# kkoutini/PaSST

Measured on AMD Instinct MI355X. Metric: clips/s (10s@32k) fwd+bwd passt_s, higher is better.
Workload: dtype bf16; 1 GPU; passt_s_swa_p16_128_ap476 train step (mel front end + mixup + fwd + BCE + bwd + adamw), 768/12/12, 474 tokens (s_patchout_t=40,f=4), random-init weights; global_batch=64, per_gpu_batch=64, parallelism=dp1, gemm_launch=persistent, 256 workgroups, input=waveform (B,1,320000) f32 resident in HBM

## Files before the change

### passt_amd/csrc/layernorm.hip

```cpp
#include <algorithm>
#include <cstdlib>

#include "pa_common.h"

namespace pa {

static constexpr int LN_MAXV = 8;
static constexpr int LN_BWD_BLOCKS = 1024;

__device__ __forceinline__ float4 ldrow4(const float* p) {
    return *(const float4*)p;
}
template <typename T> __device__ __forceinline__ void store4(T* p, const float4& v);
template <> __device__ __forceinline__ void store4<float>(float* p, const float4& v) {
    *(float4*)p = v;
}
template <> __device__ __forceinline__ void store4<bf16>(bf16* p, const float4& v) {
    bf16x4 o; o[0] = (bf16)v.x; o[1] = (bf16)v.y; o[2] = (bf16)v.z; o[3] = (bf16)v.w;
    *(bf16x4*)p = o;
}
template <typename T> __device__ __forceinline__ float4 load4(const T* p);
template <> __device__ __forceinline__ float4 load4<float>(const float* p) { return ldrow4(p); }
template <> __device__ __forceinline__ float4 load4<bf16>(const bf16* p) {
    const bf16x4 v = *(const bf16x4*)p;
    return make_float4((float)v[0], (float)v[1], (float)v[2], (float)v[3]);
}

template <typename T, int MAXV>
__global__ __launch_bounds__(256) void ln_fwd_kernel(const float* __restrict__ x, const float* __restrict__ gamma,
                                                     const float* __restrict__ beta, T* __restrict__ y,
                                                     float* __restrict__ mean, float* __restrict__ rstd,
                                                     int M, int D, float eps) {
    const int lane = threadIdx.x & 63;
    const int row = blockIdx.x * 4 + (threadIdx.x >> 6);
    if (row >= M) return;
    const int nv = D >> 2;
    const float* xr = x + (int64_t)row * D;
    float4 v[MAXV];
    float s = 0.f;
#pragma unroll
    for (int i = 0; i < MAXV; ++i) {
        const int c = lane + 64 * i;
        if (c < nv) { v[i] = ldrow4(xr + 4 * c); s += (v[i].x + v[i].y) + (v[i].z + v[i].w); }
    }
    const float mu = wave_sum(s) / (float)D;
    float s2 = 0.f;
#pragma unroll
    for (int i = 0; i < MAXV; ++i) {
        const int c = lane + 64 * i;
        if (c < nv) {
            const float a = v[i].x - mu, b = v[i].y - mu, cc = v[i].z - mu, d = v[i].w - mu;
            s2 += (a * a + b * b) + (cc * cc + d * d);
        }
    }
    const float r = rsqrtf(wave_sum(s2) / (float)D + eps);
    if (lane == 0) {
        if (mean) mean[row] = mu;
        if (rstd) rstd[row] = r;
    }
    T* yr = y + (int64_t)row * D;
#pragma unroll
    for (int i = 0; i < MAXV; ++i) {
        const int c = lane + 64 * i;
        if (c < nv) {
            const float4 g = *(const float4*)(gamma + 4 * c), b = *(const float4*)(beta + 4 * c);
            float4 o;
            o.x = (v[i].x - mu) * r * g.x + b.x; o.y = (v[i].y - mu) * r * g.y + b.y;
            o.z = (v[i].z - mu) * r * g.z + b.z; o.w = (v[i].w - mu) * r * g.w + b.w;
            store4<T>(yr + 4 * c, o);
        }
    }
}

template <typename T, int MAXV, bool ADD2>
__device__ __forceinline__ void ln_bwd_body(const T* __restrict__ dy, const float* __restrict__ x,
                                                     const float* __restrict__ gamma, const float* __restrict__ mean,
                                                     const float* __restrict__ rstd, const float* __restrict__ dres,
                                                     const float* __restrict__ dres2,
                                                     float* __restrict__ dx, T* __restrict__ dx_lp,
                                                     float* __restrict__ ws, int M, int D, float* red) {
    const int lane = threadIdx.x & 63, wave = threadIdx.x >> 6;
    const int nv = D >> 2;
    float4 g[MAXV], ag[MAXV], ab[MAXV], ac[MAXV];
#pragma unroll
    for (int i = 0; i < MAXV; ++i) {
        const int c = lane + 64 * i;
        g[i] = c < nv ? *(const float4*)(gamma + 4 * c) : make_float4(0, 0, 0, 0);
        ag[i] = make_float4(0, 0, 0, 0);
        ab[i] = make_float4(0, 0, 0, 0);
        ac[i] = make_float4(0, 0, 0, 0);
    }
    for (int row = blockIdx.x * 4 + wave; row < M; row += gridDim.x * 4) {
        const float mu = mean[row], r = rstd[row];
        const int64_t base = (int64_t)row * D;
        float4 xh[MAXV], gy[MAXV];
        float s1 = 0.f, s2 = 0.f;
#pragma unroll
        for (int i = 0; i < MAXV; ++i) {
            const int c = lane + 64 * i;
            if (c < nv) {
                const float4 xv = ldrow4(x + base + 4 * c);
                const float4 d = load4<T>(dy + base + 4 * c);
                xh[i] = make_float4((xv.x - mu) * r, (xv.y - mu) * r, (xv.z - mu) * r, (xv.w - mu) * r);
                gy[i] = make_float4(d.x * g[i].x, d.y * g[i].y, d.z * g[i].z, d.w * g[i].w);
                s1 += (gy[i].x + gy[i].y) + (gy[i].z + gy[i].w);
                s2 += (gy[i].x * xh[i].x + gy[i].y * xh[i].y) + (gy[i].z * xh[i].z + gy[i].w * xh[i].w);
                ag[i].x += d.x * xh[i].x; ag[i].y += d.y * xh[i].y; ag[i].z += d.z * xh[i].z; ag[i].w += d.w * xh[i].w;
                ab[i].x += d.x; ab[i].y += d.y; ab[i].z += d.z; ab[i].w += d.w;
            }
        }
        const float c1 = wave_sum(s1) / (float)D, c2 = wave_sum(s2) / (float)D;
#pragma unroll
        for (int i = 0; i < MAXV; ++i) {
            const int c = lane + 64 * i;
            if (c < nv) {
                float4 o;
                o.x = r * (gy[i].x - c1 - xh[i].x * c2); o.y = r * (gy[i].y - c1 - xh[i].y * c2);
                o.z = r * (gy[i].z - c1 - xh[i].z * c2); o.w = r * (gy[i].w - c1 - xh[i].w * c2);
                if (dres) {
                    const float4 dr = ldrow4(dres + base + 4 * c);
                    o.x += dr.x; o.y += dr.y; o.z += dr.z; o.w += dr.w;
                }
                if (ADD2) {
                    const float4 dr = ldrow4(dres2 + base + 4 * c);
                    o.x += dr.x; o.y += dr.y; o.z += dr.z; o.w += dr.w;
                }
                {
                    *(float4*)(dx + base + 4 * c) = o;
                }
                if (dx_lp) store4<T>(dx_lp + base + 4 * c, o);
                ac[i].x += o.x; ac[i].y += o.y; ac[i].z += o.z; ac[i].w += o.w;
            }
        }
    }
#pragma unroll
    for (int i = 0; i < MAXV; ++i) {
        const int c = lane + 64 * i;
        if (c < nv) {
            *(float4*)(red + (wave * 3 + 0) * D + 4 * c) = ag[i];
            *(float4*)(red + (wave * 3 + 1) * D + 4 * c) = ab[i];
            *(float4*)(red + (wave * 3 + 2) * D + 4 * c) = ac[i];
        }
    }
    __syncthreads();
    for (int k = threadIdx.x; k < 3 * D; k += 256) {
        const int which = k / D, c = k - which * D;
        float s = 0.f;
#pragma unroll
        for (int w = 0; w < 4; ++w) s += red[(w * 3 + which) * D + c];
        ws[(int64_t)blockIdx.x * 3 * D + k] = s;
    }
}

template <typename T, int MAXV>
__global__ __launch_bounds__(256) void ln_bwd_kernel(const T* __restrict__ dy, const float* __restrict__ x,
                                                     const float* __restrict__ gamma, const float* __restrict__ mean,
                                                     const float* __restrict__ rstd, const float* __restrict__ dres,
                                                     float* __restrict__ dx, T* __restrict__ dx_lp,
                                                     float* __restrict__ ws, int M, int D) {
    extern __shared__ __attribute__((aligned(16))) float red[];
    ln_bwd_body<T, MAXV, false>(dy, x, gamma, mean, rstd, dres, nullptr, dx, dx_lp, ws, M, D, red);
}

template <typename T, int MAXV>
__global__ __launch_bounds__(256) void ln_bwd2_kernel(const T* __restrict__ dy, const float* __restrict__ x,
                                                      const float* __restrict__ gamma, const float* __restrict__ mean,
                                                      const float* __restrict__ rstd, const float* __restrict__ dres,
                                                      const float* __restrict__ dres2,
                                                      float* __restrict__ dx, T* __restrict__ dx_lp,
                                                      float* __restrict__ ws, int M, int D) {
    extern __shared__ __attribute__((aligned(16))) float red[];
    ln_bwd_body<T, MAXV, true>(dy, x, gamma, mean, rstd, dres, dres2, dx, dx_lp, ws, M, D, red);
}

__global__ __launch_bounds__(256) void ln_bwd_reduce_kernel(const float* __restrict__ ws, int nblk, int D,
                                                            float* __restrict__ dgamma, float* __restrict__ dbeta,
                                                            float* __restrict__ dcol, int accumulate) {
    __shared__ float red[16][17];
    const int cx = threadIdx.x & 15, ry = threadIdx.x >> 4;
    const int k = blockIdx.x * 16 + cx;
    const int nk = dcol ? 3 * D : 2 * D;
    float s = 0.f, s1 = 0.f, s2 = 0.f, s3 = 0.f;
    if (k < nk) {
        int b = ry;
        for (; b + 48 < nblk; b += 64) {
            s += ws[(int64_t)b * 3 * D + k];
            s1 += ws[(int64_t)(b + 16) * 3 * D + k];
            s2 += ws[(int64_t)(b + 32) * 3 * D + k];
            s3 += ws[(int64_t)(b + 48) * 3 * D + k];
        }
        for (; b < nblk; b += 16) s += ws[(int64_t)b * 3 * D + k];
    }
    s = (s + s1) + (s2 + s3);
    red[ry][cx] = s;
    __syncthreads();
    if (ry == 0 && k < nk) {
        s = 0.f;
#pragma unroll
        for (int y = 0; y < 16; ++y) s += red[y][cx];
        float* out = k < D ? dgamma + k : (k < 2 * D ? dbeta + (k - D) : dcol + (k - 2 * D));
        *out = (accumulate ? *out : 0.f) + s;
    }
}

}

using namespace pa;

extern "C" int pa_layernorm_fwd(const float* x, const float* gamma, const float* beta, void* y, int dtype,
                                float* mean, float* rstd, int M, int D, float eps, void* stream) {
    if (!x || !gamma || !beta || !y || M <= 0 || D <= 0) return PA_EINVAL;
    if (D % 4 || D > LN_MAXV * 256) return PA_EUNSUPPORTED;
    dim3 grid((unsigned)cdiv(M, 4));
    if (dtype != PA_BF16 && dtype != PA_F32) return PA_EINVAL;
    const int nvl = (int)cdiv(D, 256);
#define PA_LN_FWD(V)                                                                                              \
    do {                                                                                                          \
        if (dtype == PA_BF16) hipLaunchKernelGGL((ln_fwd_kernel<bf16, V>), grid, dim3(256), 0, (hipStream_t)stream, x, gamma, beta, (bf16*)y, mean, rstd, M, D, eps); \
        else hipLaunchKernelGGL((ln_fwd_kernel<float, V>), grid, dim3(256), 0, (hipStream_t)stream, x, gamma, beta, (float*)y, mean, rstd, M, D, eps); \
    } while (0)
    if (nvl <= 1) PA_LN_FWD(1); else if (nvl == 2) PA_LN_FWD(2); else if (nvl == 3) PA_LN_FWD(3);
    else if (nvl == 4) PA_LN_FWD(4); else PA_LN_FWD(8);
#undef PA_LN_FWD
    return check_launch();
}

static int ln_bwd_blocks(int M) {
    static const int cap = [] { const char* e = getenv("PA_LN_BWD_BLOCKS"); return e && atoi(e) > 0 ? atoi(e) : LN_BWD_BLOCKS; }();
    static const int rpw = [] { const char* e = getenv("PA_LN_BWD_ROWS_PER_WAVE"); return e && atoi(e) > 0 ? atoi(e) : 2; }();
    return (int)std::max<int64_t>(1, std::min<int64_t>(cap, cdiv(M, 4 * rpw)));
}

extern "C" int64_t pa_layernorm_bwd_ws_floats(int M, int D) { return (int64_t)ln_bwd_blocks(M) * 3 * D; }

extern "C" int pa_layernorm_bwd_rows(int M) { return M > 0 ? ln_bwd_blocks(M) : 0; }

static int ln_bwd_launch(const void* dy, int dtype, const float* x, const float* gamma, const float* mean, const float* rstd,
                         const float* dres, const float* dres2, float* dx, void* dx_lp, float* ws, int M, int D, hipStream_t st);

extern "C" int pa_layernorm_bwd_partial(const void* dy, int dtype, const float* x, const float* gamma,
                                        const float* mean, const float* rstd, const float* dres, float* dx,
                                        void* dx_lp, float* ws, int M, int D, void* stream) {
    if (!dy || !x || !gamma || !mean || !rstd || !dx || !ws || M <= 0 || D <= 0) return PA_EINVAL;
    if (D % 4 || D > LN_MAXV * 256) return PA_EUNSUPPORTED;
    if (dtype != PA_BF16 && dtype != PA_F32) return PA_EINVAL;
    return ln_bwd_launch(dy, dtype, x, gamma, mean, rstd, dres, nullptr, dx, dx_lp, ws, M, D, (hipStream_t)stream);
}

extern "C" int pa_layernorm_bwd2_partial(const void* dy, int dtype, const float* x, const float* gamma,
                                         const float* mean, const float* rstd, const float* dres, const float* dres2,
                                         float* dx, void* dx_lp, float* ws, int M, int D, void* stream) {
    if (!dy || !x || !gamma || !mean || !rstd || !dx || !ws || M <= 0 || D <= 0) return PA_EINVAL;
    if (D % 4 || D > LN_MAXV * 256) return PA_EUNSUPPORTED;
    if (dtype != PA_BF16 && dtype != PA_F32) return PA_EINVAL;
    return ln_bwd_launch(dy, dtype, x, gamma, mean, rstd, dres, dres2, dx, dx_lp, ws, M, D, (hipStream_t)stream);
}

static int ln_bwd_finish(const void* dy, int dtype, const float* x, const float* gamma, const float* mean, const float* rstd,
                         const float* dres, const float* dres2, float* dx, void* dx_lp, float* dgamma, float* dbeta, float* dcolsum,
                         int accumulate, float* ws, int M, int D, void* stream) {
    if (!dy || !x || !gamma || !mean || !rstd || !dx || !dgamma || !dbeta || !ws || M <= 0 || D <= 0) return PA_EINVAL;
    if (D % 4 || D > LN_MAXV * 256) return PA_EUNSUPPORTED;
    if (dtype != PA_BF16 && dtype != PA_F32) return PA_EINVAL;
    hipStream_t st = (hipStream_t)stream;
    int rc = ln_bwd_launch(dy, dtype, x, gamma, mean, rstd, dres, dres2, dx, dx_lp, ws, M, D, st);
    if (rc) return rc;
    hipLaunchKernelGGL(ln_bwd_reduce_kernel, dim3((unsigned)cdiv(3 * D, 16)), dim3(256), 0, st, ws, ln_bwd_blocks(M), D, dgamma, dbeta, dcolsum, accumulate);
    return check_launch();
}

extern "C" int pa_layernorm_bwd2(const void* dy, int dtype, const float* x, const float* gamma,
                                 const float* mean, const float* rstd, const float* dres, const float* dres2, float* dx,
                                 void* dx_lp, float* dgamma, float* dbeta, float* dcolsum, int accumulate, float* ws,
                                 int M, int D, void* stream) {
    return ln_bwd_finish(dy, dtype, x, gamma, mean, rstd, dres, dres2, dx, dx_lp, dgamma, dbeta, dcolsum, accumulate, ws, M, D, stream);
}

extern "C" int pa_layernorm_bwd(const void* dy, int dtype, const float* x, const float* gamma,
                                const float* mean, const float* rstd, const float* dres, float* dx,
                                void* dx_lp, float* dgamma, float* dbeta, float* dcolsum, int accumulate, float* ws,
                                int M, int D, void* stream) {
    return ln_bwd_finish(dy, dtype, x, gamma, mean, rstd, dres, nullptr, dx, dx_lp, dgamma, dbeta, dcolsum, accumulate, ws, M, D, stream);
}

static int ln_bwd_launch(const void* dy, int dtype, const float* x, const float* gamma, const float* mean, const float* rstd,
                         const float* dres, const float* dres2, float* dx, void* dx_lp, float* ws, int M, int D, hipStream_t st) {
    const int nblk = ln_bwd_blocks(M);
    const size_t lds = (size_t)12 * D * sizeof(float);
    const int nvl = (int)cdiv(D, 256);
#define PA_LN_BWD_T(T, V)                                                                                         \
    do {                                                                                                          \
        if (dres2) hipLaunchKernelGGL((ln_bwd2_kernel<T, V>), dim3(nblk), dim3(256), lds, st, (const T*)dy, x, gamma, mean, rstd, dres, dres2, dx, (T*)dx_lp, ws, M, D); \
        else hipLaunchKernelGGL((ln_bwd_kernel<T, V>), dim3(nblk), dim3(256), lds, st, (const T*)dy, x, gamma, mean, rstd, dres, dx, (T*)dx_lp, ws, M, D); \
    } while (0)
#define PA_LN_BWD(V)                                                                                              \
    do {                                                                                                          \
        if (dtype == PA_BF16) PA_LN_BWD_T(bf16, V); else PA_LN_BWD_T(float, V);                                   \
    } while (0)
    if (nvl <= 1) PA_LN_BWD(1); else if (nvl == 2) PA_LN_BWD(2); else if (nvl == 3) PA_LN_BWD(3);
    else if (nvl == 4) PA_LN_BWD(4); else PA_LN_BWD(8);
#undef PA_LN_BWD
#undef PA_LN_BWD_T
    return check_launch();
}
```

Baseline: 2927 clips/s.

## Add persistent prefetching LayerNorm forward and lookahead backward for D=768

For D=768 (three float4 per lane), the forward LayerNorm becomes a persistent grid sized to resident blocks. Each wave caches gamma and beta in registers and prefetches the next row's input while it normalizes the current one. The backward gains a FULL specialization with no bounds checks. For bf16 without a second residual, it prefetches the next row's dy, mean and rstd, and loads the residual gradient early. The aim is to hide memory latency in these bandwidth-bound kernels, at the cost of more registers and possibly lower occupancy.

```diff
diff --git a/passt_amd/csrc/layernorm.hip b/passt_amd/csrc/layernorm.hip
--- a/passt_amd/csrc/layernorm.hip
+++ b/passt_amd/csrc/layernorm.hip
@@ -25,12 +25,93 @@
     const bf16x4 v = *(const bf16x4*)p;
     return make_float4((float)v[0], (float)v[1], (float)v[2], (float)v[3]);
 }
+template <typename T> struct raw4;
+template <> struct raw4<float> { typedef float4 type; };
+template <> struct raw4<bf16> { typedef bf16x4 type; };
+template <typename T> __device__ __forceinline__ typename raw4<T>::type ldraw4(const T* p) { return *(const typename raw4<T>::type*)p; }
+__device__ __forceinline__ float4 widen4(const float4& v) { return v; }
+__device__ __forceinline__ float4 widen4(const bf16x4& v) { return make_float4((float)v[0], (float)v[1], (float)v[2], (float)v[3]); }
+
+static constexpr int LN_STREAM_V = 3;
+
+template <typename T, int MAXV>
+__device__ __forceinline__ void ln_fwd_stream_body(const float* __restrict__ x, const float* __restrict__ gamma,
+                                                   const float* __restrict__ beta, T* __restrict__ y,
+                                                   float* __restrict__ mean, float* __restrict__ rstd,
+                                                   int M, int D, float eps) {
+    const int lane = threadIdx.x & 63;
+    const int stride = (int)gridDim.x * 4;
+    int row = blockIdx.x * 4 + __builtin_amdgcn_readfirstlane(threadIdx.x >> 6);
+    if (row >= M) return;
+    const int nv = D >> 2;
+    float4 g[MAXV], b[MAXV], nx[MAXV];
+    {
+        const float* xr = x + (int64_t)row * D;
+#pragma unroll
+        for (int i = 0; i < MAXV; ++i) {
+            const int c = lane + 64 * i;
+            if (c < nv) { nx[i] = ldrow4(xr + 4 * c); g[i] = *(const float4*)(gamma + 4 * c); b[i] = *(const float4*)(beta + 4 * c); }
+        }
+    }
+    for (;;) {
+        const bool more = (int64_t)row + stride < M;
+        float4 v[MAXV];
+        float s = 0.f;
+#pragma unroll
+        for (int i = 0; i < MAXV; ++i) v[i] = nx[i];
+        if (more) {
+            const float* xn = x + ((int64_t)row + stride) * D;
+#pragma unroll
+            for (int i = 0; i < MAXV; ++i) {
+                const int c = lane + 64 * i;
+                if (c < nv) nx[i] = ldrow4(xn + 4 * c);
+            }
+        }
+#pragma unroll
+        for (int i = 0; i < MAXV; ++i) {
+            const int c = lane + 64 * i;
+            if (c < nv) s += (v[i].x + v[i].y) + (v[i].z + v[i].w);
+        }
+        const float mu = wave_sum(s) / (float)D;
+        float s2 = 0.f;
+#pragma unroll
+        for (int i = 0; i < MAXV; ++i) {
+            const int c = lane + 64 * i;
+            if (c < nv) {
+                const float a = v[i].x - mu, bb = v[i].y - mu, cc = v[i].z - mu, d = v[i].w - mu;
+                s2 += (a * a + bb * bb) + (cc * cc + d * d);
+            }
+        }
+        const float r = rsqrtf(wave_sum(s2) / (float)D + eps);
+        if (lane == 0) {
+            if (mean) mean[row] = mu;
+            if (rstd) rstd[row] = r;
+        }
+        T* yr = y + (int64_t)row * D;
+#pragma unroll
+        for (int i = 0; i < MAXV; ++i) {
+            const int c = lane + 64 * i;
+            if (c < nv) {
+                float4 o;
+                o.x = (v[i].x - mu) * r * g[i].x + b[i].x; o.y = (v[i].y - mu) * r * g[i].y + b[i].y;
+                o.z = (v[i].z - mu) * r * g[i].z + b[i].z; o.w = (v[i].w - mu) * r * g[i].w + b[i].w;
+                store4<T>(yr + 4 * c, o);
+            }
+        }
+        if (!more) break;
+        row += stride;
+    }
+}
 
 template <typename T, int MAXV>
 __global__ __launch_bounds__(256) void ln_fwd_kernel(const float* __restrict__ x, const float* __restrict__ gamma,
                                                      const float* __restrict__ beta, T* __restrict__ y,
                                                      float* __restrict__ mean, float* __restrict__ rstd,
                                                      int M, int D, float eps) {
+    if constexpr (MAXV == LN_STREAM_V) {
+        ln_fwd_stream_body<T, MAXV>(x, gamma, beta, y, mean, rstd, M, D, eps);
+        return;
+    }
     const int lane = threadIdx.x & 63;
     const int row = blockIdx.x * 4 + (threadIdx.x >> 6);
     if (row >= M) return;
@@ -72,35 +153,63 @@
     }
 }
 
-template <typename T, int MAXV, bool ADD2>
+template <typename T, int MAXV, bool ADD2, bool FULL>
 __device__ __forceinline__ void ln_bwd_body(const T* __restrict__ dy, const float* __restrict__ x,
                                                      const float* __restrict__ gamma, const float* __restrict__ mean,
                                                      const float* __restrict__ rstd, const float* __restrict__ dres,
                                                      const float* __restrict__ dres2,
                                                      float* __restrict__ dx, T* __restrict__ dx_lp,
                                                      float* __restrict__ ws, int M, int D, float* red) {
-    const int lane = threadIdx.x & 63, wave = threadIdx.x >> 6;
+    const int lane = threadIdx.x & 63, wave = __builtin_amdgcn_readfirstlane(threadIdx.x >> 6);
     const int nv = D >> 2;
     float4 g[MAXV], ag[MAXV], ab[MAXV], ac[MAXV];
 #pragma unroll
     for (int i = 0; i < MAXV; ++i) {
         const int c = lane + 64 * i;
-        g[i] = c < nv ? *(const float4*)(gamma + 4 * c) : make_float4(0, 0, 0, 0);
+        g[i] = (FULL || c < nv) ? *(const float4*)(gamma + 4 * c) : make_float4(0, 0, 0, 0);
         ag[i] = make_float4(0, 0, 0, 0);
         ab[i] = make_float4(0, 0, 0, 0);
         ac[i] = make_float4(0, 0, 0, 0);
     }
-    for (int row = blockIdx.x * 4 + wave; row < M; row += gridDim.x * 4) {
-        const float mu = mean[row], r = rstd[row];
+    constexpr bool LA = FULL && sizeof(T) == 2 && !ADD2;
+    typedef typename raw4<T>::type R;
+    const int stride = (int)gridDim.x * 4;
+    float nmu = 0.f, nr = 0.f;
+    R nd[MAXV];
+    if (LA) {
+        const int row = blockIdx.x * 4 + wave;
+        if (row < M) {
+            nmu = mean[row]; nr = rstd[row];
+#pragma unroll
+            for (int i = 0; i < MAXV; ++i) nd[i] = ldraw4<T>(dy + (int64_t)row * D + 4 * (lane + 64 * i));
+        }
+    }
+    for (int row = blockIdx.x * 4 + wave; row < M; row += stride) {
         const int64_t base = (int64_t)row * D;
+        float mu, r;
+        R dv[MAXV];
+        if (LA) {
+            mu = nmu; r = nr;
+#pragma unroll
+            for (int i = 0; i < MAXV; ++i) dv[i] = nd[i];
+            const int64_t nrow = (int64_t)row + stride;
+            if (nrow < M) {
+                nmu = mean[nrow]; nr = rstd[nrow];
+#pragma unroll
+                for (int i = 0; i < MAXV; ++i) nd[i] = ldraw4<T>(dy + nrow * D + 4 * (lane + 64 * i));
+            }
+        } else {
+            mu = mean[row]; r = rstd[row];
+        }
         float4 xh[MAXV], gy[MAXV];
         float s1 = 0.f, s2 = 0.f;
 #pragma unroll
         for (int i = 0; i < MAXV; ++i) {
             const int c = lane + 64 * i;
-            if (c < nv) {
+            if (FULL || c < nv) {
                 const float4 xv = ldrow4(x + base + 4 * c);
-                const float4 d = load4<T>(dy + base + 4 * c);
+                if (!LA) dv[i] = ldraw4<T>(dy + base + 4 * c);
+                const float4 d = widen4(dv[i]);
                 xh[i] = make_float4((xv.x - mu) * r, (xv.y - mu) * r, (xv.z - mu) * r, (xv.w - mu) * r);
                 gy[i] = make_float4(d.x * g[i].x, d.y * g[i].y, d.z * g[i].z, d.w * g[i].w);
                 s1 += (gy[i].x + gy[i].y) + (gy[i].z + gy[i].w);
@@ -110,18 +219,25 @@
             }
         }
         const float c1 = wave_sum(s1) / (float)D, c2 = wave_sum(s2) / (float)D;
-#pragma unroll
-        for (int i = 0; i < MAXV; ++i) {
-            const int c = lane + 64 * i;
-            if (c < nv) {
+        float4 dr1[MAXV];
+        if (FULL && dres) {
+#pragma unroll
+            for (int i = 0; i < MAXV; ++i) dr1[i] = ldrow4(dres + base + 4 * (lane + 64 * i));
+        }
+#pragma unroll
+        for (int i = 0; i < MAXV; ++i) {
+            const int c = lane + 64 * i;
+            if (FULL || c < nv) {
                 float4 o;
                 o.x = r * (gy[i].x - c1 - xh[i].x * c2); o.y = r * (gy[i].y - c1 - xh[i].y * c2);
                 o.z = r * (gy[i].z - c1 - xh[i].z * c2); o.w = r * (gy[i].w - c1 - xh[i].w * c2);
                 if (dres) {
-                    const float4 dr = ldrow4(dres + base + 4 * c);
+#pragma clang fp contract(off)
+                    const float4 dr = FULL ? dr1[i] : ldrow4(dres + base + 4 * c);
                     o.x += dr.x; o.y += dr.y; o.z += dr.z; o.w += dr.w;
                 }
                 if (ADD2) {
+#pragma clang fp contract(off)
                     const float4 dr = ldrow4(dres2 + base + 4 * c);
                     o.x += dr.x; o.y += dr.y; o.z += dr.z; o.w += dr.w;
                 }
@@ -136,7 +252,7 @@
 #pragma unroll
     for (int i = 0; i < MAXV; ++i) {
         const int c = lane + 64 * i;
-        if (c < nv) {
+        if (FULL || c < nv) {
             *(float4*)(red + (wave * 3 + 0) * D + 4 * c) = ag[i];
             *(float4*)(red + (wave * 3 + 1) * D + 4 * c) = ab[i];
             *(float4*)(red + (wave * 3 + 2) * D + 4 * c) = ac[i];
@@ -159,7 +275,10 @@
                                                      float* __restrict__ dx, T* __restrict__ dx_lp,
                                                      float* __restrict__ ws, int M, int D) {
     extern __shared__ __attribute__((aligned(16))) float red[];
-    ln_bwd_body<T, MAXV, false>(dy, x, gamma, mean, rstd, dres, nullptr, dx, dx_lp, ws, M, D, red);
+    if constexpr (MAXV == LN_STREAM_V) {
+        if (D == MAXV * 256) { ln_bwd_body<T, MAXV, false, true>(dy, x, gamma, mean, rstd, dres, nullptr, dx, dx_lp, ws, M, D, red); return; }
+    }
+    ln_bwd_body<T, MAXV, false, false>(dy, x, gamma, mean, rstd, dres, nullptr, dx, dx_lp, ws, M, D, red);
 }
 
 template <typename T, int MAXV>
@@ -170,7 +289,10 @@
                                                       float* __restrict__ dx, T* __restrict__ dx_lp,
                                                       float* __restrict__ ws, int M, int D) {
     extern __shared__ __attribute__((aligned(16))) float red[];
-    ln_bwd_body<T, MAXV, true>(dy, x, gamma, mean, rstd, dres, dres2, dx, dx_lp, ws, M, D, red);
+    if constexpr (MAXV == LN_STREAM_V) {
+        if (D == MAXV * 256) { ln_bwd_body<T, MAXV, true, true>(dy, x, gamma, mean, rstd, dres, dres2, dx, dx_lp, ws, M, D, red); return; }
+    }
+    ln_bwd_body<T, MAXV, true, false>(dy, x, gamma, mean, rstd, dres, dres2, dx, dx_lp, ws, M, D, red);
 }
 
 __global__ __launch_bounds__(256) void ln_bwd_reduce_kernel(const float* __restrict__ ws, int nblk, int D,
@@ -207,6 +329,19 @@
 
 using namespace pa;
 
+template <typename T> static int64_t ln_resident_blocks() {
+    static int n[64] = {0};
+    int dev = 0;
+    if (hipGetDevice(&dev) != hipSuccess || dev < 0 || dev >= 64) return 256 * 8;
+    if (n[dev] == 0) {
+        int cus = 0, per_cu = 0;
+        if (hipDeviceGetAttribute(&cus, hipDeviceAttributeMultiprocessorCount, dev) != hipSuccess || cus <= 0) cus = 256;
+        if (hipOccupancyMaxActiveBlocksPerMultiprocessor(&per_cu, ln_fwd_kernel<T, LN_STREAM_V>, 256, 0) != hipSuccess || per_cu <= 0) per_cu = 8;
+        n[dev] = cus * per_cu;
+    }
+    return n[dev];
+}
+
 extern "C" int pa_layernorm_fwd(const float* x, const float* gamma, const float* beta, void* y, int dtype,
                                 float* mean, float* rstd, int M, int D, float eps, void* stream) {
     if (!x || !gamma || !beta || !y || M <= 0 || D <= 0) return PA_EINVAL;
@@ -219,7 +354,17 @@
         if (dtype == PA_BF16) hipLaunchKernelGGL((ln_fwd_kernel<bf16, V>), grid, dim3(256), 0, (hipStream_t)stream, x, gamma, beta, (bf16*)y, mean, rstd, M, D, eps); \
         else hipLaunchKernelGGL((ln_fwd_kernel<float, V>), grid, dim3(256), 0, (hipStream_t)stream, x, gamma, beta, (float*)y, mean, rstd, M, D, eps); \
     } while (0)
-    if (nvl <= 1) PA_LN_FWD(1); else if (nvl == 2) PA_LN_FWD(2); else if (nvl == 3) PA_LN_FWD(3);
+    if (nvl <= 1) PA_LN_FWD(1); else if (nvl == 2) PA_LN_FWD(2);
+    else if (nvl == LN_STREAM_V) {
+        hipStream_t st = (hipStream_t)stream;
+        if (dtype == PA_BF16) {
+            dim3 pg((unsigned)std::min<int64_t>(grid.x, ln_resident_blocks<bf16>()));
+            hipLaunchKernelGGL((ln_fwd_kernel<bf16, LN_STREAM_V>), pg, dim3(256), 0, st, x, gamma, beta, (bf16*)y, mean, rstd, M, D, eps);
+        } else {
+            dim3 pg((unsigned)std::min<int64_t>(grid.x, ln_resident_blocks<float>()));
+            hipLaunchKernelGGL((ln_fwd_kernel<float, LN_STREAM_V>), pg, dim3(256), 0, st, x, gamma, beta, (float*)y, mean, rstd, M, D, eps);
+        }
+    }
     else if (nvl == 4) PA_LN_FWD(4); else PA_LN_FWD(8);
 #undef PA_LN_FWD
     return check_launch();
```

New measurement: 2954 clips/s (median of 6 runs). Within noise of the previous version (+0.9%).
